# zzzqzhou/RAM-DSIR

Hardware: AMD Instinct MI355X
Metric: images/sec (seg+rec+RAM step) (higher is better)
Workload: dtype bf16; 1 GPU; Fundus target0 --ram --rec --consistency kd, batch 8=[2,3,3] per GPU, 400x400x3; dataset=fundus, consistency=kd, global_batch=8, parallelism=dp1, process_group=none (single process), hipgraph=False, streams=3, lanes_verified=True, ram_pipelined=True, launch=rd_run_list (one native call per step)

## Files before the change

### ram-dsir_amd/csrc/bn.hip

```cpp
#include "common.h"
#include "../../include/ramdsir.h"
#include "bn_fin.h"

namespace {

__global__ __launch_bounds__(64 * RD_MAX_GROUPS) void bn_finalize_fwd_kernel(const rd_bn_fwd_t p) {
    __shared__ float s_mean[RD_MAX_GROUPS], s_unb[RD_MAX_GROUPS], s_rm[RD_MAX_GROUPS], s_rv[RD_MAX_GROUPS];
    const int c = blockIdx.x, lane = threadIdx.x & 63;
    const int g = __builtin_amdgcn_readfirstlane(threadIdx.x >> 6);
    long long nbt_v[RD_MAX_GROUPS];
    if (c == 0 && threadIdx.x == 0 && p.training) {
#pragma unroll
        for (int i = 0; i < RD_MAX_GROUPS; ++i) nbt_v[i] = (i < p.G && p.num_batches_tracked[i]) ? *p.num_batches_tracked[i] : 0;
    }
    double s1 = 0.0, s2 = 0.0;
    if (p.training) {
        for (int k = lane; k < RD_STAT_SLOTS; k += 64) {
            s1 += p.stats[((size_t)(g * RD_STAT_SLOTS + k) * p.C + c) * 2 + 0];
            s2 += p.stats[((size_t)(g * RD_STAT_SLOTS + k) * p.C + c) * 2 + 1];
        }
    }
    const float cbias = p.conv_bias ? p.conv_bias[c] : 0.f;
    const float gam = p.gamma[g][c], bet = p.beta[g][c];
    const bool has_run = p.running_mean[g] != nullptr;
// ... 77 lines not shown
    __syncthreads();
    if ((int)threadIdx.x >= p.G) return;
    const int i = threadIdx.x;
    float* dgp = p.dgamma[i];
    float* dbp = p.dbeta[i];
    bool fg = dgp != nullptr, fb = dbp != nullptr;
    for (int j = 0; j < i; ++j) {
        fg = fg && p.dgamma[j] != dgp;
        fb = fb && p.dbeta[j] != dbp;
    }
    float a = fg ? dgp[c] : 0.f, b = fb ? dbp[c] : 0.f;
    for (int j = i; j < p.G; ++j) {
        if (p.dgamma[j] == dgp) a += s_s2[j];
        if (p.dbeta[j] == dbp) b += s_s1[j];
    }
    if (fg) dgp[c] = a;
    if (fb) dbp[c] = b;
}

__device__ __forceinline__ double block_sum_d(double v, double* s_tmp) {
    v = wave_sum_d(v);
    __syncthreads();
    if ((threadIdx.x & 63) == 0) s_tmp[threadIdx.x >> 6] = v;
    __syncthreads();
    double r = 0.0;
    for (int i = 0; i < (int)(blockDim.x >> 6); ++i) r += s_tmp[i];
    return r;
}

__global__ __launch_bounds__(256) void gn_finalize_fwd_kernel(const rd_bn_fwd_t p) {
    __shared__ double s_tmp[4];
    const int g = blockIdx.x;
    const double cnt = (double)p.count[g];
    double S1 = 0.0, S2 = 0.0;
    for (int c = threadIdx.x; c < p.C; c += blockDim.x) {
        double s1 = 0.0, s2 = 0.0;
        for (int k = 0; k < RD_STAT_SLOTS; ++k) {
            s1 += p.stats[((size_t)(g * RD_STAT_SLOTS + k) * p.C + c) * 2 + 0];
            s2 += p.stats[((size_t)(g * RD_STAT_SLOTS + k) * p.C + c) * 2 + 1];
        }
        const double b = p.conv_bias ? (double)p.conv_bias[c] : 0.0;
        S1 += s1 + cnt * b;
        S2 += s2 + 2.0 * b * s1 + cnt * b * b;
    }
    S1 = block_sum_d(S1, s_tmp);
    S2 = block_sum_d(S2, s_tmp);
    const double n = cnt * (double)p.C;
    const double m = S1 / n;
    double vard = S2 / n - m * m;
    if (vard < 0.0) vard = 0.0;
    const float mean = (float)m, invstd = 1.0f / sqrtf((float)vard + p.eps);
    for (int c = threadIdx.x; c < p.C; c += blockDim.x) {
        const float sc = p.gamma[g][c] * invstd;
        p.scale[g * p.C + c] = sc;
        p.shift[g * p.C + c] = p.beta[g][c] - mean * sc;
        p.mean[g * p.C + c] = mean;
        p.invstd[g * p.C + c] = invstd;
    }
}

__global__ __launch_bounds__(256) void gn_finalize_bwd_kernel(const rd_bn_bwd_t p) {
    __shared__ double s_tmp[4];
    constexpr int CPT = 4;
    float dg[CPT], db[CPT], dcb[CPT];
#pragma unroll
    for (int j = 0; j < CPT; ++j) dg[j] = db[j] = dcb[j] = 0.f;
    for (int g = 0; g < p.G; ++g) {
        const float mu = p.mean[g * p.C], is = p.invstd[g * p.C];
        double b1[CPT], b2[CPT];
        double A = 0.0, B = 0.0;
#pragma unroll
        for (int j = 0; j < CPT; ++j) {
            const int c = threadIdx.x + j * blockDim.x;
            b1[j] = b2[j] = 0.0;
            if (c < p.C) {
                for (int k = 0; k < RD_STAT_SLOTS; ++k) {
                    b1[j] += p.bstats[((size_t)(g * RD_STAT_SLOTS + k) * p.C + c) * 2 + 0];
                    b2[j] += p.bstats[((size_t)(g * RD_STAT_SLOTS + k) * p.C + c) * 2 + 1];
                }
                const double gam = (double)p.gamma[g][c];
                b2[j] = (double)is * (b2[j] - (double)mu * b1[j]);
                A += gam * b1[j];
                B += gam * b2[j];
            }
        }
        A = block_sum_d(A, s_tmp);
        B = block_sum_d(B, s_tmp);
        const double n = (double)p.count[g] * (double)p.C;
        const float Q = (float)(-(double)is * (double)is * B / n);
        const float R = (float)(-(double)is * A / n) - Q * mu;
#pragma unroll
        for (int j = 0; j < CPT; ++j) {
            const int c = threadIdx.x + j * blockDim.x;
            if (c < p.C) {
                const float P = p.gamma[g][c] * is;
                p.P[g * p.C + c] = P;
                p.Q[g * p.C + c] = Q;
                p.R[g * p.C + c] = R;
                dg[j] += (float)b2[j];
                db[j] += (float)b1[j];
                if (p.dbias) {
                    double sz = 0.0;
                    for (int k = 0; k < RD_STAT_SLOTS; ++k) sz += p.fstats[((size_t)(g * RD_STAT_SLOTS + k) * p.C + c) * 2 + 0];
                    if (p.conv_bias) sz += (double)p.count[g] * (double)p.conv_bias[c];
                    dcb[j] += (float)((double)P * b1[j] + (double)Q * sz + (double)R * (double)p.count[g]);
                }
            }
        }
    }
#pragma unroll
    for (int j = 0; j < CPT; ++j) {
        const int c = threadIdx.x + j * blockDim.x;
        if (c < p.C) {
            if (p.dgamma[0]) p.dgamma[0][c] += dg[j];
            if (p.dbeta[0]) p.dbeta[0][c] += db[j];
            if (p.dbias) p.dbias[c] += dcb[j];
        }
    }
}

template <typename T>
__device__ __forceinline__ void ldv(const T* p, float* f) {
    Slot<T>::unpack(*reinterpret_cast<const uint4*>(p), f);
}

__device__ __forceinline__ void unshift(float s1, float s2, float k, int n, double& S1, double& S2) {
    const double kd = (double)k, nd = (double)n;
    S1 = (double)s1 + nd * kd;
    S2 = (double)s2 + 2.0 * kd * (double)s1 + nd * kd * kd;
}

template <int S>
__device__ __forceinline__ void reduce_stats_d(double (&A1)[S], double (&A2)[S], double* s_red, int SL, int sl, double* stats_gc, int C) {
    const int lane = threadIdx.x & 63;
#pragma unroll
    for (int e = 0; e < S; ++e) {
        for (int o = SL; o < 64; o <<= 1) {
            A1[e] += __shfl_xor(A1[e], o, 64);
            A2[e] += __shfl_xor(A2[e], o, 64);
        }
    }
    if (lane < SL) {
#pragma unroll
        for (int e = 0; e < S; ++e) {
            atomicAdd(&s_red[(sl * S + e) * 2 + 0], (double)A1[e]);
            atomicAdd(&s_red[(sl * S + e) * 2 + 1], (double)A2[e]);
        }
    }
    __syncthreads();
    for (int i = threadIdx.x; i < 2 * C; i += blockDim.x) atomicAdd(&stats_gc[i], s_red[i]);
}

template <typename T>
__global__ __launch_bounds__(256) void up_stats_kernel(const T* t, double* stats, T* y_out, int h, int w, int C, GroupMap gm, int nslots) {
    constexpr int S = Slot<T>::N;
    extern __shared__ double s_redd[];
    const int n = blockIdx.y, g = group_of(gm, n);
    for (int i = threadIdx.x; i < 2 * C; i += blockDim.x) s_redd[i] = 0.0;
    __syncthreads();
    const int SL = C / S;
    const int H = 2 * h, W = 2 * w;
    const int bw = w + 1, items = (h + 1) * bw * SL;
    const int sl = threadIdx.x % SL;
    float a1[S], a2[S], piv[S];
    int cnt = 0;
#pragma unroll
    for (int e = 0; e < S; ++e) a1[e] = a2[e] = piv[e] = 0.f;
    const T* b = t + (size_t)n * h * w * C + sl * S;
    for (int idx = blockIdx.x * blockDim.x + threadIdx.x; idx < items; idx += gridDim.x * blockDim.x) {
        const int blk = idx / SL;
        const int bi = blk / bw, i = bi - 1, j = blk - bi * bw - 1;
        const int r0 = max(i, 0), r1 = min(i + 1, h - 1), c0 = max(j, 0), c1 = min(j + 1, w - 1);
        float t00[S], t01[S], t10[S], t11[S];
        ldv<T>(b + ((size_t)r0 * w + c0) * C, t00);
        ldv<T>(b + ((size_t)r0 * w + c1) * C, t01);
        ldv<T>(b + ((size_t)r1 * w + c0) * C, t10);
        ldv<T>(b + ((size_t)r1 * w + c1) * C, t11);
        float u[2][2][S];
#pragma unroll
        for (int e = 0; e < S; ++e) {
            const float dt = t01[e] - t00[e], db = t11[e] - t10[e];
            const float tl = t00[e] + 0.25f * dt, tr = t00[e] + 0.75f * dt;
            const float bl = t10[e] + 0.25f * db, br = t10[e] + 0.75f * db;
            const float dl = bl - tl, dr = br - tr;
            u[0][0][e] = tl + 0.25f * dl; u[1][0][e] = tl + 0.75f * dl;
            u[0][1][e] = tr + 0.25f * dr; u[1][1][e] = tr + 0.75f * dr;
        }
#pragma unroll
        for (int dy = 0; dy < 2; ++dy) {
            const int Y = 2 * i + 1 + dy;
            if ((unsigned)Y >= (unsigned)H) continue;
#pragma unroll
            for (int dx = 0; dx < 2; ++dx) {
                const int X = 2 * j + 1 + dx;
                if ((unsigned)X >= (unsigned)W) continue;
                float* uu = u[dy][dx];
                if (y_out) {
                    const uint4 pk = Slot<T>::pack(uu);
                    *reinterpret_cast<uint4*>(y_out + ((size_t)n * H * W + (size_t)Y * W + X) * C + sl * S) = pk;
                    Slot<T>::unpack(pk, uu);
                }
                if (cnt == 0) {
#pragma unroll
                    for (int e = 0; e < S; ++e) piv[e] = uu[e];
                }
                ++cnt;
#pragma unroll
                for (int e = 0; e < S; ++e) {
                    const float d = uu[e] - piv[e];
                    a1[e] += d;
                    a2[e] += d * d;
                }
            }
        }
    }
    double A1[S], A2[S];
#pragma unroll
    for (int e = 0; e < S; ++e) unshift(a1[e], a2[e], piv[e], cnt, A1[e], A2[e]);
    const int slot = (blockIdx.x + 7 * blockIdx.y) % nslots;
    reduce_stats_d<S>(A1, A2, s_redd, SL, sl, stats + ((size_t)g * RD_STAT_SLOTS + slot) * C * 2, C);
}

template <typename T>
__global__ __launch_bounds__(256) void bn_stats_kernel(const T* x, double* stats, int HW, int C, GroupMap gm) {
    extern __shared__ double s_redd[];
    const int n = blockIdx.y, g = group_of(gm, n);
    for (int i = threadIdx.x; i < 2 * C; i += blockDim.x) s_redd[i] = 0.0;
    __syncthreads();
    const int tpb = blockDim.x / C * C;
    const int c = threadIdx.x % C;
    float a1 = 0.f, a2 = 0.f, piv = 0.f;
    int cnt = 0;
    if ((int)threadIdx.x < tpb) {
        const int ppb = tpb / C;
        for (int pix = blockIdx.x * ppb + threadIdx.x / C; pix < HW; pix += gridDim.x * ppb) {
            const float v = to_f<T>(x[((size_t)n * HW + pix) * C + c]);
            if (cnt == 0) piv = v;
            ++cnt;
            const float d = v - piv;
            a1 += d;
            a2 += d * d;
        }
    }
    double A1, A2;
    unshift(a1, a2, piv, cnt, A1, A2);
    atomicAdd(&s_redd[c * 2 + 0], A1);
    atomicAdd(&s_redd[c * 2 + 1], A2);
    __syncthreads();
    const int slot = (blockIdx.x + 7 * blockIdx.y) % RD_STAT_SLOTS;
    for (int i = threadIdx.x; i < 2 * C; i += blockDim.x)
        atomicAdd(&stats[((size_t)g * RD_STAT_SLOTS + slot) * C * 2 + i], s_redd[i]);
}

template <typename T>
__global__ __launch_bounds__(256) void pool_fwd_kernel(const T* z, const float* scale, const float* shift, float slope, T* out,
                                                       int Ho, int Wo, int C, GroupMap gm, const rdfin::FinArg fa) {
    constexpr int S = Slot<T>::N;
    extern __shared__ float s_cf[];
    rdfin::prologue(fa);
    const int n = blockIdx.y, g = group_of(gm, n);
    for (int i = threadIdx.x; i < C; i += blockDim.x) {
        s_cf[i] = scale ? scale[g * C + i] : 1.f;
        s_cf[C + i] = shift ? shift[g * C + i] : 0.f;
    }
    __syncthreads();
    const int SL = C / S, W = 2 * Wo;
    const int items = Ho * Wo * SL;
    const T* zb = z + (size_t)n * 4 * Ho * Wo * C;
    for (int idx = blockIdx.x * blockDim.x + threadIdx.x; idx < items; idx += gridDim.x * blockDim.x) {
        const int sl = idx % SL, pix = idx / SL;
        const int y = pix / Wo, x = pix - y * Wo;
        float v[4][S], best[S];
#pragma unroll
        for (int k = 0; k < 4; ++k) ldv<T>(zb + ((size_t)(2 * y + (k >> 1)) * W + 2 * x + (k & 1)) * C + sl * S, v[k]);
#pragma unroll
        for (int e = 0; e < S; ++e) {
            const float sc = s_cf[sl * S + e], sh = s_cf[C + sl * S + e];
            best[e] = act_fn(v[0][e] * sc + sh, slope);
#pragma unroll
            for (int k = 1; k < 4; ++k) best[e] = fmaxf(best[e], act_fn(v[k][e] * sc + sh, slope));
        }
        *reinterpret_cast<uint4*>(out + ((size_t)n * Ho * Wo + pix) * C + sl * S) = Slot<T>::pack(best);
    }
}

template <typename T, bool ACC>
__global__ __launch_bounds__(256) void pool_bwd_kernel(const T* gp, const T* z, const float* scale, const float* shift, float slope,
                                                       int act, T* gout, double* bstats, int Ho, int Wo, int C,
                                                       GroupMap gm, int nslots) {
    constexpr int S = Slot<T>::N;
    extern __shared__ double s_redd[];
    float* s_cf = reinterpret_cast<float*>(s_redd + 2 * C);
    const int n = blockIdx.y, g = group_of(gm, n);
    for (int i = threadIdx.x; i < 2 * C; i += blockDim.x) s_redd[i] = 0.0;
    for (int i = threadIdx.x; i < C; i += blockDim.x) {
        s_cf[i] = scale ? scale[g * C + i] : 1.f;
        s_cf[C + i] = shift ? shift[g * C + i] : 0.f;
    }
    __syncthreads();
    const int SL = C / S, W = 2 * Wo;
    const int items = Ho * Wo * SL;
    const int sl = threadIdx.x % SL;
    const T* zb = z + (size_t)n * 4 * Ho * Wo * C + sl * S;
    T* gb = gout + (size_t)n * 4 * Ho * Wo * C + sl * S;
    float b1[S], b2[S], sc[S], sh[S];
#pragma unroll
    for (int e = 0; e < S; ++e) {
        b1[e] = b2[e] = 0.f;
        sc[e] = s_cf[sl * S + e];
        sh[e] = s_cf[C + sl * S + e];
    }
    for (int idx = blockIdx.x * blockDim.x + threadIdx.x; idx < items; idx += gridDim.x * blockDim.x) {
        const int pix = idx / SL;
        const int y = pix / Wo, x = pix - y * Wo;
        float zz[4][S], gw[4][S], da[S];
        ldv<T>(gp + ((size_t)n * Ho * Wo + pix) * C + sl * S, da);
#pragma unroll
        for (int k = 0; k < 4; ++k) {
            const size_t o = ((size_t)(2 * y + (k >> 1)) * W + 2 * x + (k & 1)) * C;
            ldv<T>(zb + o, zz[k]);
            if constexpr (ACC) ldv<T>(gb + o, gw[k]);
        }
#pragma unroll
        for (int e = 0; e < S; ++e) {
            float best = act_fn(zz[0][e] * sc[e] + sh[e], slope);
            int arg = 0;
#pragma unroll
            for (int k = 1; k < 4; ++k) {
                const float a = act_fn(zz[k][e] * sc[e] + sh[e], slope);
                if (a > best) { best = a; arg = k; }
            }
#pragma unroll
            for (int k = 0; k < 4; ++k) {
                float gn = 0.f;
                if (arg == k) {
                    gn = da[e] * (act ? act_grad(zz[k][e] * sc[e] + sh[e], slope) : 1.f);
                    b1[e] += gn;
                    b2[e] += gn * zz[k][e];
                }
                gw[k][e] = ACC ? gw[k][e] + gn : gn;
            }
        }
#pragma unroll
        for (int k = 0; k < 4; ++k)
            *reinterpret_cast<uint4*>(gb + ((size_t)(2 * y + (k >> 1)) * W + 2 * x + (k & 1)) * C) = Slot<T>::pack(gw[k]);
    }
    if (!bstats) return;
    double A1[S], A2[S];
#pragma unroll
    for (int e = 0; e < S; ++e) { A1[e] = (double)b1[e]; A2[e] = (double)b2[e]; }
    const int slot = (blockIdx.x + 7 * blockIdx.y) % nslots;
    reduce_stats_d<S>(A1, A2, s_redd, SL, sl, bstats + ((size_t)g * RD_STAT_SLOTS + slot) * C * 2, C);
}

__device__ __forceinline__ void up_adjoint_1d(int y, int h, float* wy, float* A) {
    A[0] = A[1] = A[2] = 0.f;
#pragma unroll
    for (int j = 0; j < 4; ++j) {
        const int Y = 2 * y - 1 + j;
        wy[j] = 0.f;
        if (Y < 0 || Y >= 2 * h) continue;
        int i0, i1;
        float lam;
        up2_coord(Y, h, i0, i1, lam);
        const float wgt = (i0 == y ? 1.f - lam : 0.f) + (i1 == y ? lam : 0.f);
        wy[j] = wgt;
        if (wgt != 0.f) {
            A[i0 - y + 1] += wgt * (1.f - lam);
            A[i1 - y + 1] += wgt * lam;
        }
    }
}

template <typename T>
__global__ __launch_bounds__(256) void up_bwd_kernel(const T* g2, const T* t, T* dt, const float* P, const float* Q,
                                                     const float* R, int h, int w, int C, GroupMap gm, const rdfin::FinArg fa) {
    constexpr int S = Slot<T>::N;
    rdfin::prologue(fa);
    const int n = blockIdx.y, gi = group_of(gm, n);
    const int SL = C / S;
    const int items = h * w * SL;
    const int H = 2 * h, W = 2 * w;
    for (int idx = blockIdx.x * blockDim.x + threadIdx.x; idx < items; idx += gridDim.x * blockDim.x) {
        const int sl = idx % SL, pix = idx / SL;
        const int y = pix / w, x = pix - y * w;
        float wy[4], wx[4], Ay[3], Ax[3];
        up_adjoint_1d(y, h, wy, Ay);
        up_adjoint_1d(x, w, wx, Ax);
        float G[S], TU[S];
#pragma unroll
        for (int e = 0; e < S; ++e) G[e] = TU[e] = 0.f;
        const T* gb = g2 + (size_t)n * H * W * C + sl * S;
        const T* tb = t + (size_t)n * h * w * C + sl * S;
        uint4 gq[4][4], tq[3][3];
#pragma unroll
        for (int j = 0; j < 4; ++j) {
            const int Yc = min(max(2 * y - 1 + j, 0), H - 1);
#pragma unroll
            for (int k = 0; k < 4; ++k) {
                const int Xc = min(max(2 * x - 1 + k, 0), W - 1);
                gq[j][k] = *reinterpret_cast<const uint4*>(gb + ((size_t)Yc * W + Xc) * C);
            }
        }
#pragma unroll
        for (int a = 0; a < 3; ++a) {
            const int yc = min(max(y + a - 1, 0), h - 1);
#pragma unroll
            for (int b = 0; b < 3; ++b) {
                const int xc = min(max(x + b - 1, 0), w - 1);
                tq[a][b] = *reinterpret_cast<const uint4*>(tb + ((size_t)yc * w + xc) * C);
            }
        }
#pragma unroll
        for (int j = 0; j < 4; ++j)
#pragma unroll
            for (int k = 0; k < 4; ++k) {
                const float wgt = wy[j] * wx[k];
                float v[S];
                Slot<T>::unpack(gq[j][k], v);
#pragma unroll
                for (int e = 0; e < S; ++e) G[e] += wgt * v[e];
            }
#pragma unroll
        for (int a = 0; a < 3; ++a)
#pragma unroll
            for (int b = 0; b < 3; ++b) {
                const float cf = Ay[a] * Ax[b];
                float v[S];
                Slot<T>::unpack(tq[a][b], v);
#pragma unroll
                for (int e = 0; e < S; ++e) TU[e] += cf * v[e];
            }
        const float Wsum = (wy[0] + wy[1] + wy[2] + wy[3]) * (wx[0] + wx[1] + wx[2] + wx[3]);
        float o[S];
#pragma unroll
        for (int e = 0; e < S; ++e) {
            const int c = gi * C + sl * S + e;
            o[e] = P[c] * G[e] + Q[c] * TU[e] + R[c] * Wsum;
        }
        *reinterpret_cast<uint4*>(dt + ((size_t)(n * h + y) * w + x) * C + sl * S) = Slot<T>::pack(o);
    }
}

template <typename T>
__global__ void nchw_to_nhwc_kernel(const float* x, T* y, int N, int C, int H, int W, int Cs) {
    const size_t total = (size_t)N * C * H * W;
    for (size_t i = (size_t)blockIdx.x * blockDim.x + threadIdx.x; i < total; i += (size_t)gridDim.x * blockDim.x) {
        const int c = i % C;
        const size_t pix = i / C;
        const int xw = pix % W, yh = (pix / W) % H, n = pix / ((size_t)W * H);
        y[pix * Cs + c] = from_f<T>(x[(((size_t)n * C + c) * H + yh) * W + xw]);
    }
}

template <typename T>
__global__ void nhwc_to_nchw_kernel(const T* z, float* y, const float* scale, const float* shift, int act, float slope,
                                    int N, int C, int H, int W, GroupMap gm) {
    const size_t total = (size_t)N * C * H * W;
    for (size_t i = (size_t)blockIdx.x * blockDim.x + threadIdx.x; i < total; i += (size_t)gridDim.x * blockDim.x) {
        const int xw = i % W, yh = (i / W) % H, c = (i / ((size_t)W * H)) % C, n = i / ((size_t)W * H * C);
        float v = to_f<T>(z[(((size_t)n * H + yh) * W + xw) * C + c]);
        if (scale) {
            const int g = group_of(gm, n);
            v = v * scale[g * C + c] + shift[g * C + c];
            if (act) v = act_fn(v, slope);
        }
        y[i] = v;
    }
}

template <typename T>
__global__ __launch_bounds__(256) void grad_in_kernel(const float* dy, const T* z, T* gout, const float* scale,
                                                      const float* shift, double* bstats, int act, float slope,
                                                      int accumulate, int C, int H, int W, GroupMap gm) {
    extern __shared__ double s_red[];
    const int n = blockIdx.y, g = group_of(gm, n);
    for (int i = threadIdx.x; i < 2 * C; i += blockDim.x) s_red[i] = 0.0;
    __syncthreads();
    const int HW = H * W;
    const int p0 = blockIdx.x * 64;
    for (int i = threadIdx.x; i < 64 * C; i += blockDim.x) {
        const int c = i / 64, pp = p0 + (i % 64);
        float gn = 0.f, zz = 0.f;
        if (pp < HW) {
            const size_t zi = ((size_t)n * HW + pp) * C + c;
            zz = z ? to_f<T>(z[zi]) : 0.f;
            float m = 1.f;
            if (act && scale) m = act_grad(zz * scale[g * C + c] + shift[g * C + c], slope);
            gn = dy[((size_t)n * C + c) * HW + pp] * m;
            gout[zi] = from_f<T>(accumulate ? to_f<T>(gout[zi]) + gn : gn);
        }
        float a = wave_sum(gn), b = wave_sum(gn * zz);
        if ((threadIdx.x & 63) == 0) {
            atomicAdd(&s_red[c * 2 + 0], (double)a);
            atomicAdd(&s_red[c * 2 + 1], (double)b);
        }
    }
    __syncthreads();
    if (bstats) {
        const int slot = (blockIdx.x + 7 * blockIdx.y) % RD_STAT_SLOTS;
        for (int i = threadIdx.x; i < 2 * C; i += blockDim.x) atomicAdd(&bstats[((size_t)g * RD_STAT_SLOTS + slot) * C * 2 + i], s_red[i]);
    }
}

template <typename T>
__global__ __launch_bounds__(256) void colsum_kernel(const T* x, float* partial, int64_t npix, int C, int Cs) {
    float acc[8];
#pragma unroll
    for (int c = 0; c < 8; ++c) acc[c] = 0.f;
    for (int64_t i = (int64_t)blockIdx.x * blockDim.x + threadIdx.x; i < npix; i += (int64_t)gridDim.x * blockDim.x)
#pragma unroll
        for (int c = 0; c < 8; ++c)
            if (c < C) acc[c] += to_f<T>(x[i * Cs + c]);
    __shared__ float s[4][8];
#pragma unroll
    for (int c = 0; c < 8; ++c) {
        const float v = wave_sum(acc[c]);
        if ((threadIdx.x & 63) == 0) s[threadIdx.x >> 6][c] = v;
    }
    __syncthreads();
    if (threadIdx.x < C) partial[blockIdx.x * 8 + threadIdx.x] = s[0][threadIdx.x] + s[1][threadIdx.x] + s[2][threadIdx.x] + s[3][threadIdx.x];
}

__global__ __launch_bounds__(64) void colsum_final_kernel(const float* partial, float* out, int nblocks, int C, float beta) {
    const int c = blockIdx.x;
    float s = 0.f;
    for (int b = threadIdx.x; b < nblocks; b += 64) s += partial[b * 8 + c];
    s = wave_sum(s);
    if (threadIdx.x == 0) out[c] = (beta != 0.f ? beta * out[c] : 0.f) + s;
}

template <typename T, bool TWO>
__global__ __launch_bounds__(256) void bn_apply_kernel(const T* x, const T* x2, T* out, const float* a, const float* b, const float* c,
                                                       float slope, int HW, int C, GroupMap gm) {
    constexpr int S = Slot<T>::N;
    const int n = blockIdx.y, g = group_of(gm, n);
    const int SL = C / S;
    const size_t base = (size_t)n * HW * C;
    const int items = HW * SL;
    for (int idx = blockIdx.x * blockDim.x + threadIdx.x; idx < items; idx += gridDim.x * blockDim.x) {
        const int sl = idx % SL;
        float ca[S], cb[S], cc[S];
#pragma unroll
        for (int e = 0; e < S; ++e) {
            ca[e] = a[g * C + sl * S + e];
            cc[e] = c[g * C + sl * S + e];
            cb[e] = TWO ? b[g * C + sl * S + e] : 0.f;
        }
        float v[S], w[S];
        const size_t off = base + (size_t)idx * S;
        Slot<T>::unpack(*reinterpret_cast<const uint4*>(x + off), v);
        if constexpr (TWO) {
            Slot<T>::unpack(*reinterpret_cast<const uint4*>(x2 + off), w);
#pragma unroll
            for (int e = 0; e < S; ++e) v[e] = act_fn(ca[e] * v[e] + cb[e] * w[e] + cc[e], slope);
        } else {
#pragma unroll
            for (int e = 0; e < S; ++e) v[e] = act_fn(ca[e] * v[e] + cc[e], slope);
        }
        *reinterpret_cast<uint4*>(out + off) = Slot<T>::pack(v);
    }
}

GroupMap host_gm(int G, const int32_t* gs) {
    GroupMap gm;
    gm.G = G;
    for (int i = 0; i <= RD_MAX_GROUPS; ++i) gm.gs[i] = (gs && i <= G) ? gs[i] : 0;
    return gm;
}

int grid_for(size_t total, int per_block = 256, int cap = 4096) {
    size_t b = (total + per_block - 1) / per_block;
    if (b > (size_t)cap) b = cap;
    if (b < 1) b = 1;
    return (int)b;
}

}

extern "C" {

int rd_bn_finalize_fwd(const rd_bn_fwd_t* p, void* stream) {
    if (!p || p->G < 1 || p->G > RD_MAX_GROUPS) return -1;
    rd_launch(bn_finalize_fwd_kernel, dim3(p->C), dim3(64 * p->G), 0, (hipStream_t)stream, *p);
    return (int)hipGetLastError();
}

int rd_bn_finalize_bwd(const rd_bn_bwd_t* p, void* stream) {
    if (!p || p->G < 1 || p->G > RD_MAX_GROUPS) return -1;
    rd_launch(bn_finalize_bwd_kernel, dim3(p->C), dim3(64 * p->G), 0, (hipStream_t)stream, *p);
    return (int)hipGetLastError();
}

int rd_gn_finalize_fwd(const rd_bn_fwd_t* p, void* stream) {
    if (!p || p->G < 1 || p->G > RD_MAX_GROUPS || p->C < 1) return -1;
    rd_launch(gn_finalize_fwd_kernel, dim3(p->G), dim3(256), 0, (hipStream_t)stream, *p);
    return (int)hipGetLastError();
}

int rd_gn_finalize_bwd(const rd_bn_bwd_t* p, void* stream) {
    if (!p || p->G < 1 || p->G > RD_MAX_GROUPS || p->C < 1 || p->C > 1024) return -1;
    rd_launch(gn_finalize_bwd_kernel, dim3(1), dim3(256), 0, (hipStream_t)stream, *p);
    return (int)hipGetLastError();
}

int rd_up_stats(const void* t, double* stats, void* y_out, int N, int h, int w, int C, int G, const int32_t* gstart_host, int dtype,
                int stat_slots, void* stream) {
    const int S = dtype == RD_BF16 ? 8 : 4;
    if (C % S || 256 % (C / S) || stat_slots < 0 || stat_slots > RD_STAT_SLOTS) return -2;
    const int nslots = stat_slots > 0 ? stat_slots : RD_STAT_SLOTS;
    const GroupMap gm = host_gm(G, gstart_host);
    const int items = (h + 1) * (w + 1) * (C / S);
    static const int us_per = rd_switch("RD_UPS_PER", 2);
    int bx = grid_for(items, 256 * us_per, 4096);
    dim3 grid(bx, N);
    if (dtype == RD_BF16)
        rd_launch(up_stats_kernel<bf16_t>, grid, dim3(256), 2 * C * sizeof(double), (hipStream_t)stream,
                           (const bf16_t*)t, stats, (bf16_t*)y_out, h, w, C, gm, nslots);
    else
        rd_launch(up_stats_kernel<float>, grid, dim3(256), 2 * C * sizeof(double), (hipStream_t)stream,
                           (const float*)t, stats, (float*)y_out, h, w, C, gm, nslots);
    return (int)hipGetLastError();
}

int rd_bn_stats(const void* x, double* stats, int N, int H, int W, int C, int G, const int32_t* gstart_host, int dtype, void* stream) {
    if (!x || !stats || C < 1 || C > 256) return -2;
    if (G < 1 || G > RD_MAX_GROUPS) return -1;
    const GroupMap gm = host_gm(G, gstart_host);
    const int ppb = 256 / C;
    const int bx = grid_for(H * W, ppb * 16, 2048);
    dim3 grid(bx, N);
    if (dtype == RD_BF16)
        rd_launch(bn_stats_kernel<bf16_t>, grid, dim3(256), 2 * C * sizeof(double), (hipStream_t)stream, (const bf16_t*)x, stats, H * W, C, gm);
    else
        rd_launch(bn_stats_kernel<float>, grid, dim3(256), 2 * C * sizeof(double), (hipStream_t)stream, (const float*)x, stats, H * W, C, gm);
    return (int)hipGetLastError();
}

int rd_pool_fwd(const void* z, const float* scale, const float* shift, float slope, void* out, int N, int Ho, int Wo, int C, int G,
                const int32_t* gstart_host, int dtype, const rd_bn_fwd_t* fin, int fin_flags, void* stream) {
    const int S = dtype == RD_BF16 ? 8 : 4;
    if (!z || !out || C % S || C > 1024) return -2;
    if (G < 1 || G > RD_MAX_GROUPS) return -1;
    rdfin::FinArg fa;
    rdfin::no_arg(fa);
    if (fin) {
        rd_src_t s;
        memset(&s, 0, sizeof(s));
        s.fin = fin;
        s.fin_flags = fin_flags;
        s.mode = RD_SRC_AFFACT;
        s.C = C;
        if (!scale || !shift || fin->scale != scale || fin->shift != shift || rdfin::make_arg(fa, &s, 1)) return -3;
    }
    const GroupMap gm = host_gm(G, gstart_host);
    dim3 grid(grid_for((size_t)Ho * Wo * (C / S), 256 * 4, 2048), N);
    if (dtype == RD_BF16)
        rd_launch(pool_fwd_kernel<bf16_t>, grid, dim3(256), 2 * C * sizeof(float), (hipStream_t)stream, (const bf16_t*)z, scale, shift,
                           slope, (bf16_t*)out, Ho, Wo, C, gm, fa);
    else
        rd_launch(pool_fwd_kernel<float>, grid, dim3(256), 2 * C * sizeof(float), (hipStream_t)stream, (const float*)z, scale, shift,
                           slope, (float*)out, Ho, Wo, C, gm, fa);
    return (int)hipGetLastError();
}

int rd_pool_bwd(const void* gp, const void* z, const float* scale, const float* shift, float slope, int act, void* g, int accumulate,
                double* bstats, int N, int Ho, int Wo, int C, int G, const int32_t* gstart_host, int dtype, int stat_slots, void* stream) {
    const int S = dtype == RD_BF16 ? 8 : 4;
    if (!gp || !z || !g || C % S || C > 1024 || 256 % (C / S) || stat_slots < 0 || stat_slots > RD_STAT_SLOTS) return -2;
    const int nslots = stat_slots > 0 ? stat_slots : RD_STAT_SLOTS;
    if (G < 1 || G > RD_MAX_GROUPS) return -1;
    const GroupMap gm = host_gm(G, gstart_host);
    dim3 grid(grid_for((size_t)Ho * Wo * (C / S), 256 * 4, 2048), N);
    const size_t lds = 2 * C * sizeof(double) + 2 * C * sizeof(float);
    if (dtype == RD_BF16) {
        if (accumulate)
            rd_launch((pool_bwd_kernel<bf16_t, true>), grid, dim3(256), lds, (hipStream_t)stream, (const bf16_t*)gp, (const bf16_t*)z, scale,
                               shift, slope, act, (bf16_t*)g, bstats, Ho, Wo, C, gm, nslots);
        else
            rd_launch((pool_bwd_kernel<bf16_t, false>), grid, dim3(256), lds, (hipStream_t)stream, (const bf16_t*)gp, (const bf16_t*)z, scale,
                               shift, slope, act, (bf16_t*)g, bstats, Ho, Wo, C, gm, nslots);
    } else {
        if (accumulate)
            rd_launch((pool_bwd_kernel<float, true>), grid, dim3(256), lds, (hipStream_t)stream, (const float*)gp, (const float*)z, scale, shift,
                               slope, act, (float*)g, bstats, Ho, Wo, C, gm, nslots);
        else
            rd_launch((pool_bwd_kernel<float, false>), grid, dim3(256), lds, (hipStream_t)stream, (const float*)gp, (const float*)z, scale, shift,
                               slope, act, (float*)g, bstats, Ho, Wo, C, gm, nslots);
    }
    return (int)hipGetLastError();
}

int rd_bn_apply(const void* x, const void* x2, void* out, const float* a, const float* b, const float* c, float slope, int N, int H,
                int W, int C, int G, const int32_t* gstart_host, int dtype, void* stream) {
    const int S = dtype == RD_BF16 ? 8 : 4;
    if (C % S || !x || !out || !a || !c || ((x2 != nullptr) != (b != nullptr))) return -2;
    if (G < 1 || G > RD_MAX_GROUPS) return -1;
    const GroupMap gm = host_gm(G, gstart_host);
    const int items = H * W * (C / S);
    dim3 grid(grid_for(items, 256 * 4, 1024), N);
    hipStream_t st = (hipStream_t)stream;
#define RD_APPLY(T_, TWO_) rd_launch((bn_apply_kernel<T_, TWO_>), grid, dim3(256), 0, st, (const T_*)x, (const T_*)x2, (T_*)out, \
                                              a, b, c, slope, H * W, C, gm)
    if (dtype == RD_BF16) { if (x2) RD_APPLY(bf16_t, true); else RD_APPLY(bf16_t, false); }
    else { if (x2) RD_APPLY(float, true); else RD_APPLY(float, false); }
#undef RD_APPLY
    return (int)hipGetLastError();
}

int rd_up_bwd(const void* g, const void* t, void* dt, const float* P, const float* Q, const float* R, int N, int h, int w,
              int C, int G, const int32_t* gstart_host, int dtype, const rd_bn_bwd_t* fin, int fin_flags, void* stream) {
    const int S = dtype == RD_BF16 ? 8 : 4;
    if (C % S) return -2;
    rdfin::FinArg fa;
    rdfin::no_arg(fa);
    if (fin) {
        rd_src_t s;
        memset(&s, 0, sizeof(s));
        s.fin = fin;
        s.fin_flags = fin_flags;
        s.mode = RD_SRC_BNBWD;
        s.C = C;
        if (fin->P != P || fin->Q != Q || fin->R != R || rdfin::make_arg(fa, &s, 1)) return -3;
    }
    const GroupMap gm = host_gm(G, gstart_host);
    dim3 grid(grid_for((size_t)h * w * (C / S), 256, 1024), N);
    if (dtype == RD_BF16)
        rd_launch(up_bwd_kernel<bf16_t>, grid, dim3(256), 0, (hipStream_t)stream, (const bf16_t*)g, (const bf16_t*)t,
                           (bf16_t*)dt, P, Q, R, h, w, C, gm, fa);
    else
        rd_launch(up_bwd_kernel<float>, grid, dim3(256), 0, (hipStream_t)stream, (const float*)g, (const float*)t,
                           (float*)dt, P, Q, R, h, w, C, gm, fa);
    return (int)hipGetLastError();
}

int rd_nchw_to_nhwc(const float* x, void* y, int N, int C, int H, int W, int cstride, int dtype, void* stream) {
    const int Cs = cstride > 0 ? cstride : C;
    if (Cs < C) return -1;
    const size_t total = (size_t)N * C * H * W;
    if (dtype == RD_BF16)
        rd_launch(nchw_to_nhwc_kernel<bf16_t>, dim3(grid_for(total)), dim3(256), 0, (hipStream_t)stream, x, (bf16_t*)y, N, C, H, W, Cs);
    else
        rd_launch(nchw_to_nhwc_kernel<float>, dim3(grid_for(total)), dim3(256), 0, (hipStream_t)stream, x, (float*)y, N, C, H, W, Cs);
    return (int)hipGetLastError();
}

int rd_nhwc_to_nchw(const void* z, float* y, const float* scale, const float* shift, int act, float slope, int N, int C,
                    int H, int W, int G, const int32_t* gstart_host, int dtype, void* stream) {
    const size_t total = (size_t)N * C * H * W;
    const GroupMap gm = host_gm(G, gstart_host);
    if (dtype == RD_BF16)
        rd_launch(nhwc_to_nchw_kernel<bf16_t>, dim3(grid_for(total)), dim3(256), 0, (hipStream_t)stream, (const bf16_t*)z, y,
                           scale, shift, act, slope, N, C, H, W, gm);
    else
        rd_launch(nhwc_to_nchw_kernel<float>, dim3(grid_for(total)), dim3(256), 0, (hipStream_t)stream, (const float*)z, y,
                           scale, shift, act, slope, N, C, H, W, gm);
    return (int)hipGetLastError();
}

int rd_grad_in(const float* dy, const void* z, void* g, const float* scale, const float* shift, double* bstats, int act,
               float slope, int accumulate, int N, int C, int H, int W, int G, const int32_t* gstart_host, int dtype,
               void* stream) {
    const GroupMap gm = host_gm(G, gstart_host);
    dim3 grid((H * W + 63) / 64, N);
    if (dtype == RD_BF16)
        rd_launch(grad_in_kernel<bf16_t>, grid, dim3(256), 2 * C * sizeof(double), (hipStream_t)stream, dy, (const bf16_t*)z,
                           (bf16_t*)g, scale, shift, bstats, act, slope, accumulate, C, H, W, gm);
    else
        rd_launch(grad_in_kernel<float>, grid, dim3(256), 2 * C * sizeof(double), (hipStream_t)stream, dy, (const float*)z,
                           (float*)g, scale, shift, bstats, act, slope, accumulate, C, H, W, gm);
    return (int)hipGetLastError();
}

int rd_colsum(const void* x, float* out, float* partial_ws, int64_t npix, int C, int cstride, float beta, int dtype, void* stream) {
    const int Cs = cstride > 0 ? cstride : C;
    if (C > 8) return -2;
    const int nb = grid_for((size_t)npix, 256 * 4, 1024);
    if (dtype == RD_BF16)
        rd_launch(colsum_kernel<bf16_t>, dim3(nb), dim3(256), 0, (hipStream_t)stream, (const bf16_t*)x, partial_ws, npix, C, Cs);
    else
        rd_launch(colsum_kernel<float>, dim3(nb), dim3(256), 0, (hipStream_t)stream, (const float*)x, partial_ws, npix, C, Cs);
    rd_launch(colsum_final_kernel, dim3(C), dim3(64), 0, (hipStream_t)stream, partial_ws, out, nb, C, beta);
    return (int)hipGetLastError();
}

}
```

Measured before the change: 1988 images/s.

## Tile upsample backward through LDS, software-pipeline up-stats loads, register pool scales

The upsample backward kernel becomes persistent and tile-based. It stages the high-res gradient and low-res input halos in shared memory with register prefetch of the next tile, so the redundant 4x4 and 3x3 global gathers are replaced by LDS reuse. The up-stats kernel is rewritten as a persistent loop that prefetches the next item's four vector loads while computing the current one, with a grid capped by CU count. Pool forward drops the LDS scale/shift table for per-thread registers and processes two items per iteration. These changes add LDS pressure and control complexity, and they add double accumulation of partial stats per logical block.

```diff
diff --git a/ram-dsir_amd/csrc/bn.hip b/ram-dsir_amd/csrc/bn.hip
--- a/ram-dsir_amd/csrc/bn.hip
+++ b/ram-dsir_amd/csrc/bn.hip
@@ -253,8 +253,10 @@
 }
 
 template <typename T>
-__global__ __launch_bounds__(256) void up_stats_kernel(const T* t, double* stats, T* y_out, int h, int w, int C, GroupMap gm, int nslots) {
+__global__ __launch_bounds__(256) void up_stats_kernel(const T* t, double* stats, T* y_out, int h, int w, int C, GroupMap gm, int nslots,
+                                                       int lblocks) {
     constexpr int S = Slot<T>::N;
+    typedef __attribute__((ext_vector_type(4))) unsigned u32x4;
     extern __shared__ double s_redd[];
     const int n = blockIdx.y, g = group_of(gm, n);
     for (int i = threadIdx.x; i < 2 * C; i += blockDim.x) s_redd[i] = 0.0;
@@ -263,61 +265,99 @@
     const int H = 2 * h, W = 2 * w;
     const int bw = w + 1, items = (h + 1) * bw * SL;
     const int sl = threadIdx.x % SL;
+    const int stride = lblocks * 256, K = (items + stride - 1) / stride;
     float a1[S], a2[S], piv[S];
+    double A1[S], A2[S];
     int cnt = 0;
 #pragma unroll
-    for (int e = 0; e < S; ++e) a1[e] = a2[e] = piv[e] = 0.f;
+    for (int e = 0; e < S; ++e) {
+        a1[e] = a2[e] = piv[e] = 0.f;
+        A1[e] = A2[e] = 0.0;
+    }
     const T* b = t + (size_t)n * h * w * C + sl * S;
-    for (int idx = blockIdx.x * blockDim.x + threadIdx.x; idx < items; idx += gridDim.x * blockDim.x) {
-        const int blk = idx / SL;
-        const int bi = blk / bw, i = bi - 1, j = blk - bi * bw - 1;
+    auto request = [&](int idx, u32x4 (&q)[4], int& i, int& j) {
+        const int blk = min(idx, items - 1) / SL;
+        const int bi = blk / bw;
+        i = bi - 1;
+        j = blk - bi * bw - 1;
         const int r0 = max(i, 0), r1 = min(i + 1, h - 1), c0 = max(j, 0), c1 = min(j + 1, w - 1);
-        float t00[S], t01[S], t10[S], t11[S];
-        ldv<T>(b + ((size_t)r0 * w + c0) * C, t00);
-        ldv<T>(b + ((size_t)r0 * w + c1) * C, t01);
-        ldv<T>(b + ((size_t)r1 * w + c0) * C, t10);
-        ldv<T>(b + ((size_t)r1 * w + c1) * C, t11);
-        float u[2][2][S];
-#pragma unroll
-        for (int e = 0; e < S; ++e) {
-            const float dt = t01[e] - t00[e], db = t11[e] - t10[e];
-            const float tl = t00[e] + 0.25f * dt, tr = t00[e] + 0.75f * dt;
-            const float bl = t10[e] + 0.25f * db, br = t10[e] + 0.75f * db;
-            const float dl = bl - tl, dr = br - tr;
-            u[0][0][e] = tl + 0.25f * dl; u[1][0][e] = tl + 0.75f * dl;
-            u[0][1][e] = tr + 0.25f * dr; u[1][1][e] = tr + 0.75f * dr;
-        }
-#pragma unroll
-        for (int dy = 0; dy < 2; ++dy) {
-            const int Y = 2 * i + 1 + dy;
-            if ((unsigned)Y >= (unsigned)H) continue;
-#pragma unroll
-            for (int dx = 0; dx < 2; ++dx) {
-                const int X = 2 * j + 1 + dx;
-                if ((unsigned)X >= (unsigned)W) continue;
-                float* uu = u[dy][dx];
-                if (y_out) {
-                    const uint4 pk = Slot<T>::pack(uu);
-                    *reinterpret_cast<uint4*>(y_out + ((size_t)n * H * W + (size_t)Y * W + X) * C + sl * S) = pk;
-                    Slot<T>::unpack(pk, uu);
+        q[0] = *reinterpret_cast<const u32x4*>(b + ((size_t)r0 * w + c0) * C);
+        q[1] = *reinterpret_cast<const u32x4*>(b + ((size_t)r0 * w + c1) * C);
+        q[2] = *reinterpret_cast<const u32x4*>(b + ((size_t)r1 * w + c0) * C);
+        q[3] = *reinterpret_cast<const u32x4*>(b + ((size_t)r1 * w + c1) * C);
+    };
+    int lb = blockIdx.x, k = 0, idx = lb * 256 + threadIdx.x;
+    u32x4 cur[4], nxt[4];
+    int i, j, ni, nj;
+    request(idx, cur, i, j);
+    while (lb < lblocks) {
+        int nk = k + 1, nlb = lb;
+        if (nk == K) { nk = 0; nlb = lb + gridDim.x; }
+        const int nidx = nlb * 256 + threadIdx.x + nk * stride;
+        request(nidx, nxt, ni, nj);
+        if (idx < items) {
+            float t00[S], t01[S], t10[S], t11[S];
+            Slot<T>::unpack(make_uint4(cur[0].x, cur[0].y, cur[0].z, cur[0].w), t00);
+            Slot<T>::unpack(make_uint4(cur[1].x, cur[1].y, cur[1].z, cur[1].w), t01);
+            Slot<T>::unpack(make_uint4(cur[2].x, cur[2].y, cur[2].z, cur[2].w), t10);
+            Slot<T>::unpack(make_uint4(cur[3].x, cur[3].y, cur[3].z, cur[3].w), t11);
+            float u[2][2][S];
+#pragma unroll
+            for (int e = 0; e < S; ++e) {
+                const float dt = t01[e] - t00[e], db = t11[e] - t10[e];
+                const float tl = t00[e] + 0.25f * dt, tr = t00[e] + 0.75f * dt;
+                const float bl = t10[e] + 0.25f * db, br = t10[e] + 0.75f * db;
+                const float dl = bl - tl, dr = br - tr;
+                u[0][0][e] = tl + 0.25f * dl; u[1][0][e] = tl + 0.75f * dl;
+                u[0][1][e] = tr + 0.25f * dr; u[1][1][e] = tr + 0.75f * dr;
+            }
+#pragma unroll
+            for (int dy = 0; dy < 2; ++dy) {
+                const int Y = 2 * i + 1 + dy;
+                if ((unsigned)Y >= (unsigned)H) continue;
+#pragma unroll
+                for (int dx = 0; dx < 2; ++dx) {
+                    const int X = 2 * j + 1 + dx;
+                    if ((unsigned)X >= (unsigned)W) continue;
+                    float* uu = u[dy][dx];
+                    if (y_out) {
+                        const uint4 pk = Slot<T>::pack(uu);
+                        *reinterpret_cast<uint4*>(y_out + ((size_t)n * H * W + (size_t)Y * W + X) * C + sl * S) = pk;
+                        Slot<T>::unpack(pk, uu);
+                    }
+                    if (cnt == 0) {
+#pragma unroll
+                        for (int e = 0; e < S; ++e) piv[e] = uu[e];
+                    }
+                    ++cnt;
+#pragma unroll
+                    for (int e = 0; e < S; ++e) {
+                        const float d = uu[e] - piv[e];
+                        a1[e] += d;
+                        a2[e] += d * d;
+                    }
                 }
-                if (cnt == 0) {
-#pragma unroll
-                    for (int e = 0; e < S; ++e) piv[e] = uu[e];
-                }
-                ++cnt;
-#pragma unroll
-                for (int e = 0; e < S; ++e) {
-                    const float d = uu[e] - piv[e];
-                    a1[e] += d;
-                    a2[e] += d * d;
-                }
-            }
-        }
-    }
-    double A1[S], A2[S];
-#pragma unroll
-    for (int e = 0; e < S; ++e) unshift(a1[e], a2[e], piv[e], cnt, A1[e], A2[e]);
+            }
+        }
+        if (nk == 0) {
+#pragma unroll
+            for (int e = 0; e < S; ++e) {
+                double c1, c2;
+                unshift(a1[e], a2[e], piv[e], cnt, c1, c2);
+                A1[e] += c1;
+                A2[e] += c2;
+                a1[e] = a2[e] = piv[e] = 0.f;
+            }
+            cnt = 0;
+        }
+#pragma unroll
+        for (int v = 0; v < 4; ++v) cur[v] = nxt[v];
+        i = ni;
+        j = nj;
+        idx = nidx;
+        lb = nlb;
+        k = nk;
+    }
     const int slot = (blockIdx.x + 7 * blockIdx.y) % nslots;
     reduce_stats_d<S>(A1, A2, s_redd, SL, sl, stats + ((size_t)g * RD_STAT_SLOTS + slot) * C * 2, C);
 }
@@ -357,31 +397,40 @@
 __global__ __launch_bounds__(256) void pool_fwd_kernel(const T* z, const float* scale, const float* shift, float slope, T* out,
                                                        int Ho, int Wo, int C, GroupMap gm, const rdfin::FinArg fa) {
     constexpr int S = Slot<T>::N;
-    extern __shared__ float s_cf[];
     rdfin::prologue(fa);
     const int n = blockIdx.y, g = group_of(gm, n);
-    for (int i = threadIdx.x; i < C; i += blockDim.x) {
-        s_cf[i] = scale ? scale[g * C + i] : 1.f;
-        s_cf[C + i] = shift ? shift[g * C + i] : 0.f;
-    }
-    __syncthreads();
     const int SL = C / S, W = 2 * Wo;
     const int items = Ho * Wo * SL;
-    const T* zb = z + (size_t)n * 4 * Ho * Wo * C;
-    for (int idx = blockIdx.x * blockDim.x + threadIdx.x; idx < items; idx += gridDim.x * blockDim.x) {
-        const int sl = idx % SL, pix = idx / SL;
-        const int y = pix / Wo, x = pix - y * Wo;
-        float v[4][S], best[S];
-#pragma unroll
-        for (int k = 0; k < 4; ++k) ldv<T>(zb + ((size_t)(2 * y + (k >> 1)) * W + 2 * x + (k & 1)) * C + sl * S, v[k]);
-#pragma unroll
-        for (int e = 0; e < S; ++e) {
-            const float sc = s_cf[sl * S + e], sh = s_cf[C + sl * S + e];
-            best[e] = act_fn(v[0][e] * sc + sh, slope);
-#pragma unroll
-            for (int k = 1; k < 4; ++k) best[e] = fmaxf(best[e], act_fn(v[k][e] * sc + sh, slope));
-        }
-        *reinterpret_cast<uint4*>(out + ((size_t)n * Ho * Wo + pix) * C + sl * S) = Slot<T>::pack(best);
+    const int sl = threadIdx.x % SL;
+    float sc[S], sh[S];
+#pragma unroll
+    for (int e = 0; e < S; ++e) {
+        sc[e] = scale ? scale[g * C + sl * S + e] : 1.f;
+        sh[e] = shift ? shift[g * C + sl * S + e] : 0.f;
+    }
+    const T* zb = z + (size_t)n * 4 * Ho * Wo * C + sl * S;
+    T* ob = out + (size_t)n * Ho * Wo * C + sl * S;
+    const int stride = gridDim.x * blockDim.x;
+    for (int idx = blockIdx.x * blockDim.x + threadIdx.x; idx < items; idx += 2 * stride) {
+        const int pix0 = idx / SL, pix1 = min(idx + stride, items - 1) / SL;
+        const int y0 = pix0 / Wo, x0 = pix0 - y0 * Wo, y1 = pix1 / Wo, x1 = pix1 - y1 * Wo;
+        float v[2][4][S];
+#pragma unroll
+        for (int k = 0; k < 4; ++k) ldv<T>(zb + ((size_t)(2 * y0 + (k >> 1)) * W + 2 * x0 + (k & 1)) * C, v[0][k]);
+#pragma unroll
+        for (int k = 0; k < 4; ++k) ldv<T>(zb + ((size_t)(2 * y1 + (k >> 1)) * W + 2 * x1 + (k & 1)) * C, v[1][k]);
+#pragma unroll
+        for (int m = 0; m < 2; ++m) {
+            float best[S];
+#pragma unroll
+            for (int e = 0; e < S; ++e) {
+                best[e] = act_fn(v[m][0][e] * sc[e] + sh[e], slope);
+#pragma unroll
+                for (int k = 1; k < 4; ++k) best[e] = fmaxf(best[e], act_fn(v[m][k][e] * sc[e] + sh[e], slope));
+            }
+            if (m == 0 || idx + stride < items)
+                *reinterpret_cast<uint4*>(ob + (size_t)(m == 0 ? pix0 : pix1) * C) = Slot<T>::pack(best);
+        }
     }
 }
 
@@ -473,73 +522,160 @@
     }
 }
 
+constexpr int UB_TY = 8, UB_TXS = 32;
+constexpr int UB_HI_LD = 6, UB_LO_LD = 2;
+struct UpTiling {
+    int lgSG;
+    int nsg;
+    int tiles_x, tiles_y, ntiles;
+};
+
+struct UpTile { int n, sg0, y0, x0; };
+__device__ __forceinline__ UpTile up_tile(const UpTiling& tl, int tile) {
+    UpTile u;
+    const int txi = tile % tl.tiles_x;
+    tile /= tl.tiles_x;
+    const int tyi = tile % tl.tiles_y;
+    tile /= tl.tiles_y;
+    u.sg0 = (tile % tl.nsg) << tl.lgSG;
+    u.n = tile / tl.nsg;
+    u.y0 = tyi * UB_TY;
+    u.x0 = txi * (UB_TXS >> tl.lgSG);
+    return u;
+}
+
 template <typename T>
-__global__ __launch_bounds__(256) void up_bwd_kernel(const T* g2, const T* t, T* dt, const float* P, const float* Q,
-                                                     const float* R, int h, int w, int C, GroupMap gm, const rdfin::FinArg fa) {
+__global__ __launch_bounds__(256, 4) void up_bwd_kernel(const T* g2, const T* t, T* dt, const float* P, const float* Q,
+                                                        const float* R, int h, int w, int C, GroupMap gm, const UpTiling tl,
+                                                        const rdfin::FinArg fa) {
     constexpr int S = Slot<T>::N;
+    extern __shared__ uint4 s_up[];
     rdfin::prologue(fa);
-    const int n = blockIdx.y, gi = group_of(gm, n);
-    const int SL = C / S;
-    const int items = h * w * SL;
+    const int lg = tl.lgSG, SG = 1 << lg, TX = UB_TXS >> lg;
+    const int RW = (2 * TX + 2) << lg, LW = (TX + 2) << lg;
+    uint4* s_hi = s_up;
+    uint4* s_lo = s_hi + UB_HI_LD * 256;
+    float* s_pqr = reinterpret_cast<float*>(s_lo + UB_LO_LD * 256);
+    float* s_wy = s_pqr + 3 * 8 * S;
+    float* s_wx = s_wy + UB_TY * 8;
     const int H = 2 * h, W = 2 * w;
-    for (int idx = blockIdx.x * blockDim.x + threadIdx.x; idx < items; idx += gridDim.x * blockDim.x) {
-        const int sl = idx % SL, pix = idx / SL;
-        const int y = pix / w, x = pix - y * w;
-        float wy[4], wx[4], Ay[3], Ax[3];
-        up_adjoint_1d(y, h, wy, Ay);
-        up_adjoint_1d(x, w, wx, Ax);
-        float G[S], TU[S];
-#pragma unroll
-        for (int e = 0; e < S; ++e) G[e] = TU[e] = 0.f;
-        const T* gb = g2 + (size_t)n * H * W * C + sl * S;
-        const T* tb = t + (size_t)n * h * w * C + sl * S;
-        uint4 gq[4][4], tq[3][3];
-#pragma unroll
-        for (int j = 0; j < 4; ++j) {
-            const int Yc = min(max(2 * y - 1 + j, 0), H - 1);
-#pragma unroll
-            for (int k = 0; k < 4; ++k) {
-                const int Xc = min(max(2 * x - 1 + k, 0), W - 1);
-                gq[j][k] = *reinterpret_cast<const uint4*>(gb + ((size_t)Yc * W + Xc) * C);
-            }
-        }
-#pragma unroll
-        for (int a = 0; a < 3; ++a) {
-            const int yc = min(max(y + a - 1, 0), h - 1);
-#pragma unroll
-            for (int b = 0; b < 3; ++b) {
-                const int xc = min(max(x + b - 1, 0), w - 1);
-                tq[a][b] = *reinterpret_cast<const uint4*>(tb + ((size_t)yc * w + xc) * C);
-            }
-        }
-#pragma unroll
-        for (int j = 0; j < 4; ++j)
-#pragma unroll
-            for (int k = 0; k < 4; ++k) {
-                const float wgt = wy[j] * wx[k];
-                float v[S];
-                Slot<T>::unpack(gq[j][k], v);
-#pragma unroll
-                for (int e = 0; e < S; ++e) G[e] += wgt * v[e];
-            }
-#pragma unroll
-        for (int a = 0; a < 3; ++a)
-#pragma unroll
-            for (int b = 0; b < 3; ++b) {
-                const float cf = Ay[a] * Ax[b];
-                float v[S];
-                Slot<T>::unpack(tq[a][b], v);
-#pragma unroll
-                for (int e = 0; e < S; ++e) TU[e] += cf * v[e];
-            }
-        const float Wsum = (wy[0] + wy[1] + wy[2] + wy[3]) * (wx[0] + wx[1] + wx[2] + wx[3]);
-        float o[S];
-#pragma unroll
-        for (int e = 0; e < S; ++e) {
-            const int c = gi * C + sl * S + e;
-            o[e] = P[c] * G[e] + Q[c] * TU[e] + R[c] * Wsum;
-        }
-        *reinterpret_cast<uint4*>(dt + ((size_t)(n * h + y) * w + x) * C + sl * S) = Slot<T>::pack(o);
+    const int tid = threadIdx.x;
+    const int hr0 = tid / RW, hc0 = tid - hr0 * RW, hdr = 256 / RW, hdc = 256 - hdr * RW;
+    const int lr0 = tid / LW, lc0 = tid - lr0 * LW, ldr = 256 / LW, ldc = 256 - ldr * LW;
+    const int is = tid & (SG - 1), itx = (tid >> lg) & (TX - 1), ity = tid >> 5;
+    const int nch = SG * S;
+
+    typedef __attribute__((ext_vector_type(4))) unsigned u32x4;
+    u32x4 hq[UB_HI_LD], lq[UB_LO_LD];
+    float pq = 0.f, qq = 0.f, rq = 0.f;
+    int cur = -1, next = blockIdx.x;
+    while (true) {
+        const bool more = next < tl.ntiles;
+        const UpTile un = up_tile(tl, more ? next : cur);
+        if (more) {
+            const T* gb = g2 + (size_t)un.n * H * W * C + un.sg0 * S;
+            const T* tb = t + (size_t)un.n * h * w * C + un.sg0 * S;
+            int r = hr0, c = hc0;
+#pragma unroll
+            for (int i = 0; i < UB_HI_LD; ++i) {
+                const int Yc = min(max(2 * un.y0 - 1 + r, 0), H - 1), Xc = min(max(2 * un.x0 - 1 + (c >> lg), 0), W - 1);
+                hq[i] = *reinterpret_cast<const u32x4*>(gb + ((size_t)Yc * W + Xc) * C + (c & (SG - 1)) * S);
+                r += hdr;
+                c += hdc;
+                if (c >= RW) { c -= RW; ++r; }
+            }
+            r = lr0;
+            c = lc0;
+#pragma unroll
+            for (int i = 0; i < UB_LO_LD; ++i) {
+                const int yc = min(max(un.y0 - 1 + r, 0), h - 1), xc = min(max(un.x0 - 1 + (c >> lg), 0), w - 1);
+                lq[i] = *reinterpret_cast<const u32x4*>(tb + ((size_t)yc * w + xc) * C + (c & (SG - 1)) * S);
+                r += ldr;
+                c += ldc;
+                if (c >= LW) { c -= LW; ++r; }
+            }
+            const int ci = group_of(gm, un.n) * C + un.sg0 * S + min(tid, nch - 1);
+            pq = P[ci];
+            qq = Q[ci];
+            rq = R[ci];
+        }
+        if (cur >= 0) {
+            const UpTile u = up_tile(tl, cur);
+            float wy[4], wx[4], Ax[3];
+#pragma unroll
+            for (int j = 0; j < 4; ++j) { wy[j] = s_wy[ity * 8 + j]; wx[j] = s_wx[itx * 8 + j]; }
+#pragma unroll
+            for (int j = 0; j < 3; ++j) Ax[j] = s_wx[itx * 8 + 4 + j];
+            float G[S], TU[S];
+#pragma unroll
+            for (int e = 0; e < S; ++e) G[e] = TU[e] = 0.f;
+            const uint4* hb = s_hi + (2 * ity) * RW + ((2 * itx) << lg) + is;
+            const uint4* lb = s_lo + ity * LW + (itx << lg) + is;
+#pragma unroll 1
+            for (int j = 0; j < 4; ++j) {
+                const float wyj = s_wy[ity * 8 + j];
+#pragma unroll
+                for (int k = 0; k < 4; ++k) {
+                    const float wgt = wyj * wx[k];
+                    float v[S];
+                    Slot<T>::unpack(hb[j * RW + (k << lg)], v);
+#pragma unroll
+                    for (int e = 0; e < S; ++e) G[e] += wgt * v[e];
+                }
+            }
+#pragma unroll 1
+            for (int a = 0; a < 3; ++a) {
+                const float Aya = s_wy[ity * 8 + 4 + a];
+#pragma unroll
+                for (int b = 0; b < 3; ++b) {
+                    const float cf = Aya * Ax[b];
+                    float v[S];
+                    Slot<T>::unpack(lb[a * LW + (b << lg)], v);
+#pragma unroll
+                    for (int e = 0; e < S; ++e) TU[e] += cf * v[e];
+                }
+            }
+            const float Wsum = (wy[0] + wy[1] + wy[2] + wy[3]) * (wx[0] + wx[1] + wx[2] + wx[3]);
+            float o[S];
+#pragma unroll
+            for (int e = 0; e < S; ++e) {
+                const int c = is * S + e;
+                o[e] = s_pqr[c] * G[e] + s_pqr[nch + c] * TU[e] + s_pqr[2 * nch + c] * Wsum;
+            }
+            const int y = u.y0 + ity, x = u.x0 + itx;
+            if (y < h && x < w)
+                *reinterpret_cast<uint4*>(dt + ((size_t)(u.n * h + y) * w + x) * C + (u.sg0 + is) * S) = Slot<T>::pack(o);
+        }
+        if (!more) break;
+        __syncthreads();
+#pragma unroll
+        for (int i = 0; i < UB_HI_LD; ++i) reinterpret_cast<u32x4*>(s_hi)[tid + 256 * i] = hq[i];
+#pragma unroll
+        for (int i = 0; i < UB_LO_LD; ++i) reinterpret_cast<u32x4*>(s_lo)[tid + 256 * i] = lq[i];
+        if (tid < nch) {
+            s_pqr[tid] = pq;
+            s_pqr[nch + tid] = qq;
+            s_pqr[2 * nch + tid] = rq;
+        }
+        if (tid < UB_TY) {
+            float wy[4], Ay[3];
+            up_adjoint_1d(min(un.y0 + tid, h - 1), h, wy, Ay);
+#pragma unroll
+            for (int j = 0; j < 4; ++j) s_wy[tid * 8 + j] = wy[j];
+#pragma unroll
+            for (int j = 0; j < 3; ++j) s_wy[tid * 8 + 4 + j] = Ay[j];
+        } else if (tid >= 64 && tid < 64 + TX) {
+            const int q = tid - 64;
+            float wx[4], Ax[3];
+            up_adjoint_1d(min(un.x0 + q, w - 1), w, wx, Ax);
+#pragma unroll
+            for (int j = 0; j < 4; ++j) s_wx[q * 8 + j] = wx[j];
+#pragma unroll
+            for (int j = 0; j < 3; ++j) s_wx[q * 8 + 4 + j] = Ax[j];
+        }
+        __syncthreads();
+        cur = next;
+        next += gridDim.x;
     }
 }
 
@@ -713,14 +849,17 @@
     const GroupMap gm = host_gm(G, gstart_host);
     const int items = (h + 1) * (w + 1) * (C / S);
     static const int us_per = rd_switch("RD_UPS_PER", 2);
-    int bx = grid_for(items, 256 * us_per, 4096);
-    dim3 grid(bx, N);
+    const int lblocks = grid_for(items, 256 * us_per, 4096);
+    static const int per_cu = rd_switch("RD_UPS_PER_CU", 3);
+    const int cap = rd_num_cus() * per_cu / (N > 0 ? N : 1) + 1;
+    const int rounds = (lblocks + cap - 1) / cap;
+    dim3 grid((lblocks + rounds - 1) / rounds, N);
     if (dtype == RD_BF16)
         rd_launch(up_stats_kernel<bf16_t>, grid, dim3(256), 2 * C * sizeof(double), (hipStream_t)stream,
-                           (const bf16_t*)t, stats, (bf16_t*)y_out, h, w, C, gm, nslots);
+                           (const bf16_t*)t, stats, (bf16_t*)y_out, h, w, C, gm, nslots, lblocks);
     else
         rd_launch(up_stats_kernel<float>, grid, dim3(256), 2 * C * sizeof(double), (hipStream_t)stream,
-                           (const float*)t, stats, (float*)y_out, h, w, C, gm, nslots);
+                           (const float*)t, stats, (float*)y_out, h, w, C, gm, nslots, lblocks);
     return (int)hipGetLastError();
 }
 
@@ -755,12 +894,13 @@
         if (!scale || !shift || fin->scale != scale || fin->shift != shift || rdfin::make_arg(fa, &s, 1)) return -3;
     }
     const GroupMap gm = host_gm(G, gstart_host);
-    dim3 grid(grid_for((size_t)Ho * Wo * (C / S), 256 * 4, 2048), N);
+    const int SL = C / S, threads = 256 - 256 % SL;
+    dim3 grid(grid_for((size_t)Ho * Wo * SL, threads * 4, 2048), N);
     if (dtype == RD_BF16)
-        rd_launch(pool_fwd_kernel<bf16_t>, grid, dim3(256), 2 * C * sizeof(float), (hipStream_t)stream, (const bf16_t*)z, scale, shift,
+        rd_launch(pool_fwd_kernel<bf16_t>, grid, dim3(threads), 0, (hipStream_t)stream, (const bf16_t*)z, scale, shift,
                            slope, (bf16_t*)out, Ho, Wo, C, gm, fa);
     else
-        rd_launch(pool_fwd_kernel<float>, grid, dim3(256), 2 * C * sizeof(float), (hipStream_t)stream, (const float*)z, scale, shift,
+        rd_launch(pool_fwd_kernel<float>, grid, dim3(threads), 0, (hipStream_t)stream, (const float*)z, scale, shift,
                            slope, (float*)out, Ho, Wo, C, gm, fa);
     return (int)hipGetLastError();
 }
@@ -825,13 +965,26 @@
         if (fin->P != P || fin->Q != Q || fin->R != R || rdfin::make_arg(fa, &s, 1)) return -3;
     }
     const GroupMap gm = host_gm(G, gstart_host);
-    dim3 grid(grid_for((size_t)h * w * (C / S), 256, 1024), N);
+    const int SL = C / S;
+    UpTiling tl;
+    tl.lgSG = 0;
+    while (tl.lgSG < 3 && SL % (2 << tl.lgSG) == 0) ++tl.lgSG;
+    tl.nsg = SL >> tl.lgSG;
+    tl.tiles_x = (w + (UB_TXS >> tl.lgSG) - 1) / (UB_TXS >> tl.lgSG);
+    tl.tiles_y = (h + UB_TY - 1) / UB_TY;
+    const long long ntiles = (long long)N * tl.nsg * tl.tiles_y * tl.tiles_x;
+    if (N < 1 || h < 1 || w < 1 || ntiles > 0x7fffffff) return -2;
+    tl.ntiles = (int)ntiles;
+    const size_t lds = (UB_HI_LD + UB_LO_LD) * 256 * sizeof(uint4) + (3 * 8 * S + UB_TY * 8 + UB_TXS * 8) * sizeof(float);
+    static const int per_cu = rd_switch("RD_UPB_PER_CU", 4);
+    const int cap = rd_num_cus() * per_cu, rounds = (tl.ntiles + cap - 1) / cap;
+    dim3 grid((tl.ntiles + rounds - 1) / rounds);
     if (dtype == RD_BF16)
-        rd_launch(up_bwd_kernel<bf16_t>, grid, dim3(256), 0, (hipStream_t)stream, (const bf16_t*)g, (const bf16_t*)t,
-                           (bf16_t*)dt, P, Q, R, h, w, C, gm, fa);
+        rd_launch(up_bwd_kernel<bf16_t>, grid, dim3(256), lds, (hipStream_t)stream, (const bf16_t*)g, (const bf16_t*)t,
+                           (bf16_t*)dt, P, Q, R, h, w, C, gm, tl, fa);
     else
-        rd_launch(up_bwd_kernel<float>, grid, dim3(256), 0, (hipStream_t)stream, (const float*)g, (const float*)t,
-                           (float*)dt, P, Q, R, h, w, C, gm, fa);
+        rd_launch(up_bwd_kernel<float>, grid, dim3(256), lds, (hipStream_t)stream, (const float*)g, (const float*)t,
+                           (float*)dt, P, Q, R, h, w, C, gm, tl, fa);
     return (int)hipGetLastError();
 }
 
```

Result: no change. 1989 images/s, median of 2 (+0.0%).
